# nv-tlabs/vid2player3d

Measured on AMD Instinct MI355X. Metric: env-steps/sec at num_envs=8192, SMPL humanoid imitation, higher is better.
Workload: dtype f32

## Files before the change

vid2player3d_amd/csrc/physics_ll.hip:

```cpp
#include <hip/hip_runtime.h>
#include <math.h>
#include <stdlib.h>
#include <string.h>

#if !defined(V2P_LL_STRICT_MATH)
#if !defined(V2P_LL_PRECISE_SINCOS)
#define PHYS_SINCOS(x, s, c) do { (s) = __sinf(x); (c) = __cosf(x); } while (0)
#endif
#if !defined(V2P_LL_PRECISE_SQRT)
#define PHYS_SQRT(x) __builtin_amdgcn_sqrtf(x)
#endif
#if !defined(V2P_LL_PRECISE_RCP)
#define PHYS_RCP(x) __builtin_amdgcn_rcpf(x)
#endif
#endif
#include "phys_common.hpp"
#include "hull_gjk.hpp"

#if defined(V2P_LL_REGS_BUILD)
#define V2P_LL_NS ll_regs
#define V2P_LL_LAUNCHER launch_env_physics_ll_regs
#else
#define V2P_LL_NS ll_lds
#define V2P_LL_LAUNCHER launch_env_physics_ll
#endif

namespace v2p {

#include "strict_ops.inc"

typedef volatile __attribute__((address_space(3))) float lds_vfloat;
constexpr int LPE = 32;

__device__ __forceinline__ bool any64(bool p) { return __builtin_amdgcn_ballot_w64(p) != 0ull; }
__device__ __forceinline__ uint8_t flag_ld(const uint8_t* p) { return __hip_atomic_load(p, __ATOMIC_RELAXED, __HIP_MEMORY_SCOPE_SYSTEM); }
__device__ __forceinline__ void flag_st(uint8_t* p, uint8_t v) { __hip_atomic_store(p, v, __ATOMIC_RELAXED, __HIP_MEMORY_SCOPE_SYSTEM); }
__device__ __forceinline__ float cload(const float* p) { return __hip_atomic_load(p, __ATOMIC_RELAXED, __HIP_MEMORY_SCOPE_SYSTEM); }
__device__ __forceinline__ void cstore(float* p, float v) { __hip_atomic_store(p, v, __ATOMIC_RELAXED, __HIP_MEMORY_SCOPE_SYSTEM); }
typedef float f4 __attribute__((ext_vector_type(4)));
__device__ __forceinline__ void cstore4(float* p, float x, float y, float z, float w) {
    const f4 v{x, y, z, w};
    asm volatile("global_store_dwordx4 %0, %1, off sc0 sc1\n\ts_nop 1" ::"v"(p), "v"(v) : "memory");
}
__device__ __forceinline__ void cload4x2(const float* p0, const float* p1, f4& a, f4& b) {
    asm volatile("global_load_dwordx4 %0, %2, off sc0 sc1\n\tglobal_load_dwordx4 %1, %3, off sc0 sc1\n\ts_waitcnt vmcnt(0)" : "=&v"(a), "=&v"(b) : "v"(p0), "v"(p1) : "memory");
}

__device__ __forceinline__ float pull(float v, int src_lane) {
    return __int_as_float(__builtin_amdgcn_ds_bpermute(src_lane << 2, __float_as_int(v)));
}
__device__ __forceinline__ V3 pull(V3 v, int s) { return V3{pull(v.x, s), pull(v.y, s), pull(v.z, s)}; }
__device__ __forceinline__ Q4 pull(Q4 q, int s) { return Q4{pull(q.x, s), pull(q.y, s), pull(q.z, s), pull(q.w, s)}; }
__device__ __forceinline__ Sym3 pull(const Sym3& a, int s) {
    return Sym3{pull(a.xx, s), pull(a.xy, s), pull(a.xz, s), pull(a.yy, s), pull(a.yz, s), pull(a.zz, s)};
}
__device__ __forceinline__ M3 pull(const M3& a, int s) {
    M3 r;
#pragma unroll
    for (int i = 0; i < 9; ++i) r.m[i] = pull(a.m[i], s);
    return r;
}
__device__ __forceinline__ float from_next(float v) { return __int_as_float(__builtin_amdgcn_update_dpp(0, __float_as_int(v), 0x130, 0xf, 0xf, true)); }
__device__ __forceinline__ V3 from_next(V3 v) { return V3{from_next(v.x), from_next(v.y), from_next(v.z)}; }
__device__ __forceinline__ Sym3 from_next(const Sym3& a) {
    return Sym3{from_next(a.xx), from_next(a.xy), from_next(a.xz), from_next(a.yy), from_next(a.yz), from_next(a.zz)};
}
__device__ __forceinline__ M3 from_next(const M3& a) {
    M3 r;
#pragma unroll
    for (int i = 0; i < 9; ++i) r.m[i] = from_next(a.m[i]);
    return r;
}
struct ParentPull {
    int plane;
    bool chain;
    __device__ __forceinline__ float operator()(float v, bool nonchain) const {
        return pull(v, plane);
    }
    __device__ __forceinline__ V3 operator()(V3 v, bool nonchain) const {
        return V3{pull(v.x, plane), pull(v.y, plane), pull(v.z, plane)};
    }
    __device__ __forceinline__ Q4 operator()(Q4 q, bool nonchain) const {
        return Q4{pull(q.x, plane), pull(q.y, plane), pull(q.z, plane), pull(q.w, plane)};
    }
    __device__ __forceinline__ Sym3 operator()(const Sym3& a, bool nonchain) const {
        return Sym3{pull(a.xx, plane), pull(a.xy, plane), pull(a.xz, plane), pull(a.yy, plane), pull(a.yz, plane), pull(a.zz, plane)};
    }
    __device__ __forceinline__ M3 operator()(const M3& a, bool nonchain) const {
        M3 r;
#pragma unroll
        for (int i = 0; i < 9; ++i) r.m[i] = pull(a.m[i], plane);
        return r;
    }
};
__device__ __forceinline__ Sym3 operator+(const Sym3& a, const Sym3& b) {
    return Sym3{a.xx + b.xx, a.xy + b.xy, a.xz + b.xz, a.yy + b.yy, a.yz + b.yz, a.zz + b.zz};
}
__device__ __forceinline__ Sym3 mask(bool c, const Sym3& a) {
    return Sym3{c ? a.xx : 0.f, c ? a.xy : 0.f, c ? a.xz : 0.f, c ? a.yy : 0.f, c ? a.yz : 0.f, c ? a.zz : 0.f};
}
__device__ __forceinline__ V3 mask(bool c, V3 a) { return V3{c ? a.x : 0.f, c ? a.y : 0.f, c ? a.z : 0.f}; }

__device__ __forceinline__ unsigned grp_xor1(unsigned v) { return (unsigned)__builtin_amdgcn_update_dpp(0, (int)v, 0xB1, 0xf, 0xf, false); }
__device__ __forceinline__ unsigned grp_xor2(unsigned v) { return (unsigned)__builtin_amdgcn_update_dpp(0, (int)v, 0x4E, 0xf, 0xf, false); }
__device__ __forceinline__ unsigned grp_mirror(unsigned v) { return (unsigned)__builtin_amdgcn_update_dpp(0, (int)v, 0x141, 0xf, 0xf, false); }
template <bool MAX, typename F>
__device__ __forceinline__ void grp_arg_step(float& v, int& k, F xch) {
    const float ov = __uint_as_float(xch(__float_as_uint(v)));
    const int ok = (int)xch((unsigned)k);
    const bool beats = MAX ? ov > v : ov < v;
    const bool take = ok >= 0 && (k < 0 || beats || (ov == v && ok < k));
    v = take ? ov : v;
    k = take ? ok : k;
}
__device__ __forceinline__ void grp_argmin(float& v, int& k) {
    grp_arg_step<false>(v, k, grp_xor1); grp_arg_step<false>(v, k, grp_xor2); grp_arg_step<false>(v, k, grp_mirror);
}
__device__ __forceinline__ void grp_argmax(float& v, int& k) {
    grp_arg_step<true>(v, k, grp_xor1); grp_arg_step<true>(v, k, grp_xor2); grp_arg_step<true>(v, k, grp_mirror);
}
__device__ __forceinline__ float grp_fmin(float v) {
    v = fminf(v, __uint_as_float(grp_xor1(__float_as_uint(v)))); v = fminf(v, __uint_as_float(grp_xor2(__float_as_uint(v)))); v = fminf(v, __uint_as_float(grp_mirror(__float_as_uint(v))));
    return v;
}
__device__ __forceinline__ float grp_fmax(float v) {
    v = fmaxf(v, __uint_as_float(grp_xor1(__float_as_uint(v)))); v = fmaxf(v, __uint_as_float(grp_xor2(__float_as_uint(v)))); v = fmaxf(v, __uint_as_float(grp_mirror(__float_as_uint(v))));
    return v;
}
__device__ __forceinline__ unsigned grp_umin(unsigned v) {
    unsigned o = grp_xor1(v); v = o < v ? o : v; o = grp_xor2(v); v = o < v ? o : v; o = grp_mirror(v); v = o < v ? o : v;
    return v;
}
template <bool MAX, bool FAST>
__device__ __forceinline__ void grp_arg(float& v, int& k) {
    if (!FAST) {
        if (MAX) grp_argmax(v, k); else grp_argmin(v, k);
        return;
    }
    const float m = k < 0 ? (MAX ? -3.0e38f : 3.0e38f) : v;
    const float g = MAX ? grp_fmax(m) : grp_fmin(m);
    const unsigned c = grp_umin((k >= 0 && m == g) ? (unsigned)k : 0x7fffffffu);
    k = c == 0x7fffffffu ? -1 : (int)c;
    v = g;
}

#define LLSUBV(k, tv) do { if (DIAG && a.prof) { long long t_ = clock64(); if (((a.prof_heavy ? blockIdx.x < 8u : (blockIdx.x & 63) == 0)) && lane == 0) atomicAdd((unsigned long long*)&a.prof[k], (unsigned long long)(t_ - tv)); tv = t_; } } while (0)
#define LLSUB(k) LLSUBV(k, tsub)
#ifdef V2P_LL_REGS_BUILD
#define LLSUBX(k, tv) do { } while (0)
#define LLSUBX_OR(k, kparent) LLSUB(kparent)
#define V2P_LL_DIAGX false
#else
#define LLSUBX(k, tv) LLSUBV(k, tv)
#define LLSUBX_OR(k, kparent) LLSUB(k)
#define V2P_LL_DIAGX DIAG
#endif
#define LLPH(k) do { if (DIAG && a.prof) { long long t_ = clock64(); if (((a.prof_heavy ? blockIdx.x < 8u : (blockIdx.x & 63) == 0)) && lane == 0) atomicAdd((unsigned long long*)&a.prof[k], (unsigned long long)(t_ - tprev)); tprev = t_; } } while (0)

inline namespace V2P_LL_NS {
#ifndef V2P_LL_WPS
#define V2P_LL_WPS 3
#endif
#ifndef V2P_LL_WPS_BALL
#define V2P_LL_WPS_BALL 3
#endif
#ifndef V2P_LL_WPS_LIMITS
#define V2P_LL_WPS_LIMITS 3
#endif
constexpr int LL_WPB = V2P_LL_WPB;
#ifndef V2P_LL_PARK2
#define V2P_LL_PARK2 1
#endif
constexpr bool PARK2 = V2P_LL_PARK2 != 0;
#ifndef V2P_LL_PARK3
#define V2P_LL_PARK3 1
#endif
constexpr bool PARK3 = V2P_LL_PARK3 != 0;
#ifndef V2P_LL_WAIT_SLEEP
#define V2P_LL_WAIT_SLEEP 16
#endif
constexpr int PARK_TAR = 0, PARK_W0 = 3, PARK_XD0 = 6, PARK_Q = 9, PARK_X = 13, PARK_CR = 16, PARK_CB = 28, PARK_CL = 32,
              PARK_SCR = PARK3 ? 44 : 16,
              PARK_SLOTS = PARK_SCR + 1;
constexpr int ROOTLAM_FLOATS = 2 * 24;
constexpr int BL_POS = 0, BL_QUAT = 3, BL_VEL = 7, BL_ANG = 10, BL_F = 13, BL_GA = 16, BL_GGAP = 17, BL_GBIAS = 18, BL_GLAM = 19, BL_GREST = 22, BL_RK = 24,
              RK_A = 0, RK_GAP = 1, RK_BIAS = 2, RK_RL = 3, RK_N = 6, RK_LAM = 9, RK_LINK = 12, RK_REST = 13, NBREC = 5, BL_V0 = BL_RK + 16 * NBREC, BL_SLOTS = BL_V0 + 8;
constexpr int LDS_FLOATS_PER_WAVE = PARK_SLOTS * 64 + 2 * BL_SLOTS + ROOTLAM_FLOATS;
__device__ __noinline__ f4 ball_hull_distance(ConstShape* S, int v0, int nv, V3 c) {
    V3 p;
    const float d = hull_closest([&](int k) { return V3{S->hull_verts[v0 + k][0], S->hull_verts[v0 + k][1], S->hull_verts[v0 + k][2]}; }, nv, c, p);
    return f4{p.x, p.y, p.z, d};
}
template <bool LDS>
struct ContactStore;
template <>
struct ContactStore<false> {
    V3 r_[4];
    float b_[4];
    V3 l_[4];
    __device__ __forceinline__ explicit ContactStore(float*) {}
    __device__ __forceinline__ V3 cr(int c) const { return r_[c]; }
    __device__ __forceinline__ void set_cr(int c, V3 v) { r_[c] = v; }
    __device__ __forceinline__ float bias(int c) const { return b_[c]; }
    __device__ __forceinline__ void set_bias(int c, float v) { b_[c] = v; }
    __device__ __forceinline__ V3 lam(int c) const { return l_[c]; }
    __device__ __forceinline__ void set_lam(int c, V3 v) { l_[c] = v; }
};
template <>
struct ContactStore<true> {
    float* p;
    __device__ __forceinline__ explicit ContactStore(float* park) : p(park) {}
    __device__ __forceinline__ V3 cr(int c) const { return V3{p[(PARK_CR + 3 * c) * 64], p[(PARK_CR + 3 * c + 1) * 64], p[(PARK_CR + 3 * c + 2) * 64]}; }
    __device__ __forceinline__ void set_cr(int c, V3 v) { p[(PARK_CR + 3 * c) * 64] = v.x; p[(PARK_CR + 3 * c + 1) * 64] = v.y; p[(PARK_CR + 3 * c + 2) * 64] = v.z; }
    __device__ __forceinline__ float bias(int c) const { return p[(PARK_CB + c) * 64]; }
    __device__ __forceinline__ void set_bias(int c, float v) { p[(PARK_CB + c) * 64] = v; }
    __device__ __forceinline__ V3 lam(int c) const { return V3{p[(PARK_CL + 3 * c) * 64], p[(PARK_CL + 3 * c + 1) * 64], p[(PARK_CL + 3 * c + 2) * 64]}; }
    __device__ __forceinline__ void set_lam(int c, V3 v) { p[(PARK_CL + 3 * c) * 64] = v.x; p[(PARK_CL + 3 * c + 1) * 64] = v.y; p[(PARK_CL + 3 * c + 2) * 64] = v.z; }
};

__device__ __forceinline__ void vfric_frame(const V3& w0, const V3& xd0, const V3& rr, V3& t1, V3& t2) {
    const float vx = xd0.x + w0.y * rr.z - w0.z * rr.y, vy = xd0.y + w0.z * rr.x - w0.x * rr.z;
    const float s2 = vx * vx + vy * vy;
    const bool on = s2 > 1e-12f;
    const float inv = on ? rsqrtf(s2) : 0.f;
    t1 = on ? V3{vx * inv, vy * inv, 0.f} : V3{1.f, 0.f, 0.f};
    t2 = V3{-t1.y, t1.x, 0.f};
}
template <bool CONTACT, bool MULTI, bool TGS, bool DIAG, bool BALL, bool JOBS, bool LIMITS, bool VFRIC = false>
__global__ __launch_bounds__(64 * LL_WPB, DIAG ? 2 : (BALL ? V2P_LL_WPS_BALL : (LIMITS ? V2P_LL_WPS_LIMITS : V2P_LL_WPS))) void physics_ll_kernel(PhysArgs a) {
    constexpr bool OPAQUE_H = BALL || LIMITS;
    const int64_t N = a.n;
    const int lane = threadIdx.x & 63;
    const int half = lane >> 5;
    const int lb = lane & (LPE - 1);
    const bool valid = lb < NB;
    const int b = valid ? lb : 0;
    const int base = lane & LPE;
    const int nblk = JOBS ? a.job_blocks : (int)gridDim.x;
    const int jid = (int)blockIdx.x;
    const bool mono = !JOBS || jid < a.job_mono;
    const int jcut = JOBS && nblk > a.job_mono ? nblk - a.job_mono : 1;
    const int jrel = JOBS ? jid - a.job_mono : 0;
    const int sjob = mono ? 0 : jrel / jcut;
    int jpair = jrel % jcut;
    if (JOBS && !mono && a.job_interleave) {
        const int nmix = a.pl_mix > a.job_mono ? (a.pl_mix < nblk ? a.pl_mix : nblk) - a.job_mono : 0;
        const int neq = jcut - nmix, both = 2 * (nmix < neq ? nmix : neq);
        if (jpair < both) jpair = (jpair & 1) ? nmix + (jpair >> 1) : (jpair >> 1);
        else jpair = nmix < neq ? jpair : jpair - neq;
    }
    const int bid = mono ? jid : a.job_mono + jpair;
    const int64_t slot = ((int64_t)bid * LL_WPB + (threadIdx.x >> 6)) * 2 + half;
    const bool live_env = slot < N;
    const int jlen = JOBS ? a.job_len : 1;
    const int jlead = JOBS ? a.job_lead : 1;
    auto jstart = [&](int j) -> int { return j <= 0 ? 0 : jlead + (j - 1) * jlen; };
    const bool first_job = mono || sjob == 0, last_job = mono || jstart(sjob + 1) >= a.p.nsub;
    bool handed = !mono && sjob > 0;
    int* const progress = JOBS ? a.job_progress + (bid * LL_WPB + (threadIdx.x >> 6)) : nullptr;
    if constexpr (JOBS) if (!mono) {
        int done = 0;
        if (lane == 0) done = __hip_atomic_load(progress, __ATOMIC_RELAXED, __HIP_MEMORY_SCOPE_SYSTEM) >= a.job_epoch * (a.p.nsub + 1) + a.p.nsub;
        if (__builtin_amdgcn_readfirstlane(done)) {
            if (lane == 0 && half == 0) __hip_atomic_fetch_add(a.job_progress + a.job_blocks * LL_WPB + 1, 1, __ATOMIC_RELAXED, __HIP_MEMORY_SCOPE_SYSTEM);
            return;
        }
    }
    auto wait_for_predecessor = [&]() {
    if constexpr (JOBS) if (handed) {
        const int want = a.job_epoch * (a.p.nsub + 1) + sjob;
        int ok = 1;
        if (lane == 0) {
            long spins = 0;
            while (__hip_atomic_load(progress, __ATOMIC_RELAXED, __HIP_MEMORY_SCOPE_SYSTEM) < want) {
                if (spins >= a.job_timeout_spins) {
                    ok = 0;
                    __hip_atomic_fetch_add(a.job_progress + a.job_blocks * LL_WPB, 1, __ATOMIC_RELAXED, __HIP_MEMORY_SCOPE_SYSTEM);
                    break;
                }
                __builtin_amdgcn_s_sleep(V2P_LL_WAIT_SLEEP);
                ++spins;
            }
        }
        handed = __builtin_amdgcn_readfirstlane(ok) != 0;
        __builtin_amdgcn_wave_barrier();
    }
    };
    wait_for_predecessor();
    int64_t e = live_env ? slot : N - 1;
    if (a.pl_start && handed) {
        e = __hip_atomic_load(&a.pl_slot_env[live_env ? slot : N - 1], __ATOMIC_RELAXED, __HIP_MEMORY_SCOPE_SYSTEM);
    } else if (a.pl_start) {
        const int nn = (int)N, mixn = a.pl_mix;
        const int64_t sl0 = ((int64_t)bid * LL_WPB + (threadIdx.x >> 6)) * 2;
        const int s0 = (int)(sl0 < N ? sl0 : N - 1), s1 = (int)(sl0 + 1 < N ? sl0 + 1 : N - 1);
        const int r0 = s0 < 2 * mixn ? ((s0 & 1) ? nn - 1 - (s0 >> 1) : (s0 >> 1)) : s0 - mixn;
// ... 603 lines not shown
#endif
                int* const scr = (int*)(park_all + (threadIdx.x >> 6) * LDS_FLOATS_PER_WAVE + PARK_SCR * 64);
                if (near) scr[myk] = lane;
                if (DIAG && a.prof && ((a.prof_heavy ? blockIdx.x < 8u : (blockIdx.x & 63) == 0)) && lane == 0) atomicAdd((unsigned long long*)&a.prof[13], (unsigned long long)rounds);
                for (int rd = 0; rd < rounds; ++rd) {
                    const int kk = 8 * rd + grp;
                    const bool gon = kk < ntot;
                    const int src = gon ? scr[kk] : lane;
                    const M3 RL = q2mat(pull(q, src));
                    const V3 xL = pull(x, src);
                    const float r6 = RL.m[6], r7 = RL.m[7], r8 = RL.m[8], xz = xL.z;
                    const int v0L = __builtin_amdgcn_ds_bpermute(src << 2, v0), nvL = __builtin_amdgcn_ds_bpermute(src << 2, nv);
                    ConstShape* const SL = MULTI ? (ConstShape*)(a.shapes + __builtin_amdgcn_ds_bpermute(src << 2, sid)) : S;
                    auto hullv = [&](int idx) -> float4 { return make_float4(SL->hull_verts[idx][0], SL->hull_verts[idx][1], SL->hull_verts[idx][2], 0.f); };
                    const float r0 = RL.m[0], r1 = RL.m[1], r2 = RL.m[2], xx = xL.x;
                    const float r3 = RL.m[3], r4 = RL.m[4], r5 = RL.m[5], xy = xL.y;
                    const unsigned gbit = 1u << gl;
                    float4 vv[8];
#pragma unroll
                    for (int k = 0; k < 8; ++k) {
                        const int i = 8 * k + gl;
                        vv[k] = hullv(v0L + ((gon && i < nvL) ? i : 0));
                    }
                    float px[8], py[8];
                    unsigned clo = 0u, chi = 0u;
                    int k0 = -1;
                    float zmin = 0.f;
#pragma unroll
                    for (int k = 0; k < 8; ++k) {
                        const int i = 8 * k + gl;
                        const bool in = gon && i < nvL;
                        const float z = xz + r6 * vv[k].x + r7 * vv[k].y + r8 * vv[k].z;
                        px[k] = xx + r0 * vv[k].x + r1 * vv[k].y + r2 * vv[k].z;
                        py[k] = xy + r3 * vv[k].x + r4 * vv[k].y + r5 * vv[k].z;
                        const bool c = in && (z < coff);
                        const unsigned bit = c ? gbit << (8 * (k & 3)) : 0u;
                        if (k < 4) clo |= bit; else chi |= bit;
                        const bool better = c && (k0 < 0 || z < zmin);
                        k0 = better ? i : k0;
                        zmin = better ? z : zmin;
                    }
                    clo |= grp_xor1(clo); chi |= grp_xor1(chi);
                    clo |= grp_xor2(clo); chi |= grp_xor2(chi);
                    clo |= grp_mirror(clo); chi |= grp_mirror(chi);
                    grp_arg<false, FASTARG>(zmin, k0);
                    const unsigned long long cm = ((unsigned long long)chi << 32) | clo;
                    const int cntg = __popc(clo) + __popc(chi);
                    unsigned long long t = cm;
                    int s0 = t ? __ffsll((long long)t) - 1 : -1; t &= t - 1;
                    int s1 = t ? __ffsll((long long)t) - 1 : -1; t &= t - 1;
                    int s2 = t ? __ffsll((long long)t) - 1 : -1; t &= t - 1;
                    int s3 = t ? __ffsll((long long)t) - 1 : -1;
                    int ns = cntg < 4 ? cntg : 4;
                    const bool big = gon && cntg > 4;
                    if (any64(big)) {
                        if (DIAG && a.prof && ((a.prof_heavy ? blockIdx.x < 8u : (blockIdx.x & 63) == 0)) && lane == 0) atomicAdd((unsigned long long*)&a.prof[15], 1ull);
                        const int k0s = k0 < 0 ? 0 : k0;
                        const float4 u0 = hullv(v0L + k0s);
                        const float p0x = xx + r0 * u0.x + r1 * u0.y + r2 * u0.z;
                        const float p0y = xy + r3 * u0.x + r4 * u0.y + r5 * u0.z;
                        const unsigned long long remB = big ? (cm & ~(1ull << k0s)) : 0ull;
                        const unsigned blo = (unsigned)remB, bhi = (unsigned)(remB >> 32);
                        int k1 = -1;
                        float best = -1.f;
#pragma unroll
                        for (int k = 0; k < 8; ++k) {
                            const bool on = ((k < 4 ? blo : bhi) & (gbit << (8 * (k & 3)))) != 0u;
                            const float dx = px[k] - p0x, dy = py[k] - p0y;
                            const float d2 = dx * dx + dy * dy;
                            const bool take = on && (d2 > best);
                            best = take ? d2 : best;
                            k1 = take ? 8 * k + gl : k1;
                        }
                        grp_arg<true, FASTARG>(best, k1);
                        const int k1s = k1 < 0 ? 0 : k1;
                        const float4 u1 = hullv(v0L + k1s);
                        const float ex = xx + r0 * u1.x + r1 * u1.y + r2 * u1.z - p0x;
                        const float ey = xy + r3 * u1.x + r4 * u1.y + r5 * u1.z - p0y;
                        const unsigned long long remC = remB & ~(1ull << k1s);
                        const unsigned elo = (unsigned)remC, ehi = (unsigned)(remC >> 32);
                        int k2 = -1, k3 = -1;
                        float amax = 0.f, amin = 0.f;
#pragma unroll
                        for (int k = 0; k < 8; ++k) {
                            const bool on = ((k < 4 ? elo : ehi) & (gbit << (8 * (k & 3)))) != 0u;
                            const float dx = px[k] - p0x, dy = py[k] - p0y;
                            const float area = ex * dy - ey * dx;
                            const bool up = on && area > amax;
                            const bool dn = on && area < amin;
                            amax = up ? area : amax; k2 = up ? 8 * k + gl : k2;
                            amin = dn ? area : amin; k3 = dn ? 8 * k + gl : k3;
                        }
                        grp_arg<true, FASTARG>(amax, k2);
                        grp_arg<false, FASTARG>(amin, k3);
                        if (big) {
                            s0 = k0; s1 = k1;
                            s2 = k2 >= 0 ? k2 : k3;
                            s3 = k2 >= 0 ? k3 : -1;
                            ns = 2 + (k2 >= 0 ? 1 : 0) + (k3 >= 0 ? 1 : 0);
                        }
                    }
                    const int gpack = (s0 & 0x7f) | ((s1 & 0x7f) << 7) | ((s2 & 0x7f) << 14) | ((s3 & 0x7f) << 21) | (ns << 28);
                    const int got = __builtin_amdgcn_ds_bpermute(((myk & 7) << 3) << 2, gpack);
                    pack = (near && (myk >> 3) == rd) ? got : pack;
                }
            }
            LLSUB(17);
            int sel4[4];
#pragma unroll
            for (int c = 0; c < 4; ++c) {
                const int sv = (pack >> (7 * c)) & 0x7f;
                sel4[c] = sv == 0x7f ? -1 : sv;
            }
            cnt = (pack >> 28) & 7;
            if (any64(cnt > 0)) {
                const M3 R = q2mat(q);
                const float ih = 1.f / h;
#pragma unroll
                for (int c = 0; c < 4; ++c) {
                    const float4 uu = hullv(v0 + (sel4[c] < 0 ? 0 : sel4[c]));
                    const V3 crc = mul(R, V3{uu.x, uu.y, uu.z});
                    CS.set_cr(c, crc);
                    float dz = x.z + crc.z - P.rest_offset;
                    CS.set_bias(c, TGS ? dz : (dz >= 0.f ? dz * ih : fmaxf(P.erp * dz * ih, -P.max_depen)));
                }
            }
            if (a.contact_ids && last && valid && live_env && !frozen) {
#pragma unroll
                for (int c = 0; c < 4; ++c) a.contact_ids[(env_here() * NB + b) * 4 + c] = c < cnt ? b * 64 + sel4[c] : -1;
            }
            if (a.contact_ids_sub && valid && live_env && !frozen) {
#pragma unroll
                for (int c = 0; c < 4; ++c) a.contact_ids_sub[((env_here() * nsub + sub) * NB + b) * 4 + c] = c < cnt ? b * 64 + sel4[c] : -1;
            }

            LLSUB(18);
            if (PARK2 && lb == 0) {
                float lv[21];
#pragma unroll
                for (int k = 0; k < 21; ++k) lv[k] = rootlam[k];
                Lam.A = Sym3{lv[0], lv[1], lv[2], lv[3], lv[4], lv[5]};
#pragma unroll
                for (int k = 0; k < 9; ++k) Lam.B.m[k] = lv[6 + k];
                Lam.C = Sym3{lv[15], lv[16], lv[17], lv[18], lv[19], lv[20]};
            }
            auto ball_rec_mine = [&](int j) -> bool { return j < 2 ? racket_lane : lb == (int)bl[BL_RK + 16 * j + RK_LINK]; };
            bool myhull = false;
            if (BALL) {
#pragma unroll
                for (int j = 2; j < NBREC; ++j) myhull = myhull || (bl[BL_RK + 16 * j + RK_A] != 0.f && lb == (int)bl[BL_RK + 16 * j + RK_LINK]);
            }
            const bool ballhit = BALL && valid && ((racket_lane && (bl[BL_RK + RK_A] != 0.f || bl[BL_RK + 16 + RK_A] != 0.f)) || myhull);
            const bool ballground = BALL && ball_lane && bl[BL_GA] != 0.f;
            const unsigned long long tb = __ballot(valid && (cnt > 0 || ballhit));
            const unsigned m0 = (unsigned)tb, m1 = (unsigned)(tb >> 32);
            if (LIMITS && any64(limact)) {
                const V3 wv = PARK2 ? park_get3(PARK_W0) : w;
                const V3 pwv = pp(wv, true);
                const V3 om = mulT(q2mat(q), wv - pwv);
                const float mrate = P.limit_margin * PHYS_RCP(h);
                const float lscale = TGS ? PHYS_RCP(h) : 1.f;
                bool anyrow = false;
#pragma unroll
                for (int i = 0; i < 3; ++i) {
                    const float omi = i == 0 ? om.x : (i == 1 ? om.y : om.z);
                    const bool on = lsgn[i] != 0.f && lbias[i] * lscale < mrate + fmaxf(0.f, -lsgn[i] * omi);
                    if (!on) lsgn[i] = 0.f;
                    anyrow = anyrow || on;
                }
                limact = anyrow;
            }
            const unsigned long long lmb = LIMITS ? __ballot(valid && limact) : 0ull;
            const unsigned lm0 = (unsigned)lmb, lm1 = (unsigned)(lmb >> 32);
            if (DIAG && a.wave_times) { const int tt = __popc(half ? m1 : m0); tsum += tt; tmaxs = tt > tmaxs ? tt : tmaxs; }
            if (last) {
                const unsigned mine = half ? m1 : m0;
                ksum = __popc(mine);
                kdep = 0;
                for (unsigned t = mine; t; t &= t - 1) { const int dd = M.depth[__ffs(t) - 1]; kdep = dd > kdep ? dd : kdep; }
            }
            if (DIAG && a.prof && ((a.prof_heavy ? blockIdx.x < 8u : (blockIdx.x & 63) == 0)) && lane == 0) { atomicAdd((unsigned long long*)&a.prof[9], (unsigned long long)(__popc(m0) + __popc(m1))); atomicAdd((unsigned long long*)&a.prof[10], 1ull); }
            const bool sweep_on = ((m0 | m1 | lm0 | lm1) || (BALL && any64(ballground))) && P.n_iter > 0;
            if (PARK2 && !sweep_on) unpark_vel(w, xd);
            if (sweep_on) {
                int dn0 = 0, dn1 = 0;
                for (unsigned t = m0 | lm0; t; t &= t - 1) { const int dd = M.depth[__ffs(t) - 1]; dn0 = dd > dn0 ? dd : dn0; }
                for (unsigned t = m1 | lm1; t; t &= t - 1) { const int dd = M.depth[__ffs(t) - 1]; dn1 = dd > dn1 ? dd : dn1; }
                const int dneed = dn0 > dn1 ? dn0 : dn1, dmin = dn0 < dn1 ? dn0 : dn1;
                const bool insweep = dep <= (half ? dn1 : dn0);
                LLPH(4);
                for (int d = 1; d <= dneed; ++d) {
                    Blocks Lp;
                    const bool nc = (nonchain >> d) & 1;
                    Lp.A = pp(Lam.A, nc);
                    Lp.B = pp(Lam.B, nc);
                    Lp.C = pp(Lam.C, nc);
                    if (dep == d) {
                        V3 la0{Lp.A.xx, Lp.A.xy, Lp.A.xz}, la1{Lp.A.xy, Lp.A.yy, Lp.A.yz}, la2{Lp.A.xz, Lp.A.yz, Lp.A.zz};
                        M3 Gb;
                        {
                            V3 g0 = cross(la0, r) + row(Lp.B, 0), g1 = cross(la1, r) + row(Lp.B, 1), g2 = cross(la2, r) + row(Lp.B, 2);
                            Gb.m[0] = g0.x; Gb.m[1] = g0.y; Gb.m[2] = g0.z; Gb.m[3] = g1.x; Gb.m[4] = g1.y; Gb.m[5] = g1.z; Gb.m[6] = g2.x; Gb.m[7] = g2.y; Gb.m[8] = g2.z;
                        }
                        Sym3 Gc;
                        {
                            V3 q0 = cross(col(Gb, 0), r), q1 = cross(col(Gb, 1), r), q2 = cross(col(Gb, 2), r);
                            V3 n0 = cross(r, col(Lp.B, 0)), n1 = cross(r, col(Lp.B, 1)), n2 = cross(r, col(Lp.B, 2));
                            Gc.xx = Lp.C.xx + q0.x - n0.x;
                            Gc.xy = Lp.C.xy + q0.y - n1.x;
                            Gc.xz = Lp.C.xz + q0.z - n2.x;
                            Gc.yy = Lp.C.yy + q1.y - n1.y;
                            Gc.yz = Lp.C.yz + q1.z - n2.y;
                            Gc.zz = Lp.C.zz + q2.z - n2.z;
                        }
                        M3 DiM;
                        DiM.m[0] = Di.xx; DiM.m[1] = Di.xy; DiM.m[2] = Di.xz; DiM.m[3] = Di.xy; DiM.m[4] = Di.yy; DiM.m[5] = Di.yz; DiM.m[6] = Di.xz; DiM.m[7] = Di.yz; DiM.m[8] = Di.zz;
                        M3 H1, H2;
#pragma unroll
                        for (int i = 0; i < 3; ++i) {
                            V3 gai = i == 0 ? la0 : (i == 1 ? la1 : la2);
                            V3 gbi = row(Gb, i);
                            V3 gbti = col(Gb, i);
                            V3 gci = i == 0 ? V3{Gc.xx, Gc.xy, Gc.xz} : (i == 1 ? V3{Gc.xy, Gc.yy, Gc.yz} : V3{Gc.xz, Gc.yz, Gc.zz});
#pragma unroll
                            for (int j = 0; j < 3; ++j) {
                                V3 dj = col(DiM, j);
                                V3 ej = row(E, j);
                                H1.m[3 * i + j] = aug * dot(gai, dj) - dot(gbi, ej);
                                H2.m[3 * i + j] = aug * dot(gbti, dj) - dot(gci, ej);
                            }
                        }
                        M3 t;
#pragma unroll
                        for (int i = 0; i < 3; ++i)
#pragma unroll
                            for (int j = 0; j < 3; ++j) t.m[3 * i + j] = aug * dot(row(DiM, i), col(H1, j)) - dot(row(E, i), col(H2, j));
                        Lam.A = Sym3{Di.xx + t.m[0], Di.xy + 0.5f * (t.m[1] + t.m[3]), Di.xz + 0.5f * (t.m[2] + t.m[6]), Di.yy + t.m[4],
                                     Di.yz + 0.5f * (t.m[5] + t.m[7]), Di.zz + t.m[8]};
#pragma unroll
                        for (int i = 0; i < 3; ++i)
#pragma unroll
                            for (int j = 0; j < 3; ++j) {
                                V3 gcj = j == 0 ? V3{Gc.xx, Gc.xy, Gc.xz} : (j == 1 ? V3{Gc.xy, Gc.yy, Gc.yz} : V3{Gc.xz, Gc.yz, Gc.zz});
                                Lam.B.m[3 * i + j] = aug * dot(row(DiM, i), col(Gb, j)) - dot(row(E, i), gcj);
                            }
                        Lam.C = Gc;
                        if (LIMITS && limact) {
                            const Sym3 K{Lam.A.xx - 2.f * H1.m[0] + Lp.A.xx, Lam.A.xy - H1.m[1] - H1.m[3] + Lp.A.xy, Lam.A.xz - H1.m[2] - H1.m[6] + Lp.A.xz,
                                         Lam.A.yy - 2.f * H1.m[4] + Lp.A.yy, Lam.A.yz - H1.m[5] - H1.m[7] + Lp.A.yz, Lam.A.zz - 2.f * H1.m[8] + Lp.A.zz};
                            const M3 R = q2mat(Q4{park[PARK_Q * 64], park[(PARK_Q + 1) * 64], park[(PARK_Q + 2) * 64], park[(PARK_Q + 3) * 64]});
                            const V3 c0 = col(R, 0), c1 = col(R, 1), c2 = col(R, 2);
                            const V3 k0 = mul(K, c0), k1 = mul(K, c1), k2 = mul(K, c2);
                            Kd = Sym3{dot(c0, k0), dot(c0, k1), dot(c0, k2), dot(c1, k1), dot(c1, k2), dot(c2, k2)};
                        }
                    }
                }

                auto ball_dirs = [&](V3 n, V3& t1, V3& t2) {
                    t1 = cross(n, V3{0.f, 0.f, 1.f});
                    if (dot(t1, t1) < 1e-6f) t1 = cross(n, V3{1.f, 0.f, 0.f});
                    t1 = rsqrtf(dot(t1, t1)) * t1;
                    t2 = cross(n, t1);
                };
                if (PARK2) unpark_vel(w, xd);
                if (BALL && ballhit) {
                    const V3 bv{bl[BL_VEL], bl[BL_VEL + 1], bl[BL_VEL + 2]}, bw{bl[BL_ANG], bl[BL_ANG + 1], bl[BL_ANG + 2]};
                    const float ih = PHYS_RCP(h);
#pragma unroll
                    for (int j = 0; j < NBREC; ++j) {
                        lds_vfloat* rk = bl + BL_RK + 16 * j;
                        if (rk[RK_A] != 0.f && ball_rec_mine(j)) {
                            const V3 n{rk[RK_N], rk[RK_N + 1], rk[RK_N + 2]}, rl{rk[RK_RL], rk[RK_RL + 1], rk[RK_RL + 2]};
                            const float gap = rk[RK_GAP];
                            const float vn0 = dot(bv + cross(bw, -BP.radius * n) - xd - cross(w, rl), n);
                            float bias = gap >= 0.f ? gap * ih : fmaxf(P.erp * gap * ih, -P.max_depen);
                            const float rest = (vn0 < -BP.bounce_thr && gap * ih + vn0 < 0.f) ? (j < 2 ? BP.rest_racket : BP.rest_body) * vn0 : 3.0e38f;
                            bias = fminf(bias, rest);
                            rk[RK_BIAS] = bias;
                            if (TGS) rk[RK_REST] = rest;
                        }
                    }
                }
                LLPH(5);
                if (!PARK2) {
                    park_put3(PARK_W0, w);
                    park_put3(PARK_XD0, xd);
                }
                [[maybe_unused]] unsigned chain0 = 0u, chain1 = 0u;
                {
                    int prev = -1;
                    for (unsigned t = m0; t; t &= t - 1) {
                        const int nn = __ffs(t) - 1;
                        if ((int)((a.par_pack[nn / 12] >> (5 * (nn % 12))) & 31ull) == prev) chain0 |= 1u << nn;
                        prev = nn;
                    }
                    prev = -1;
                    for (unsigned t = m1; t; t &= t - 1) {
                        const int nn = __ffs(t) - 1;
                        if ((int)((a.par_pack[nn / 12] >> (5 * (nn % 12))) & 31ull) == prev) chain1 |= 1u << nn;
                        prev = nn;
                    }
                    chain0 &= ~lm0;
                    chain1 &= ~lm1;
                }
                const float hs = h / (float)P.n_iter;
                float tgs_irem = 1.f / h;
                const float tgs_pen = P.erp / hs;
                auto rowbias = [&](float v) -> float { return TGS ? (v >= 0.f ? v * tgs_irem : fmaxf(tgs_pen * v, -P.max_depen)) : v; };
                V3 un_tot{0.f, 0.f, 0.f}, un_new{0.f, 0.f, 0.f}, uf_new{0.f, 0.f, 0.f}, Dw{0.f, 0.f, 0.f}, Dv{0.f, 0.f, 0.f};
                int cur0 = 0, cur1 = 0;
                bool live0 = false, live1 = false;
                const unsigned v0 = LIMITS ? m0 | lm0 : m0, v1 = LIMITS ? m1 | lm1 : m1;
                V3 jt_new{0.f, 0.f, 0.f};
#ifdef V2P_LL_REGS_BUILD
                constexpr bool VTAB = !LIMITS && !TGS && !BALL && !DIAG;
#else
                constexpr bool VTAB = !LIMITS && !TGS && !BALL;
#endif
                constexpr bool LIVEM = VTAB;
#ifdef V2P_LL_REGS_BUILD
                constexpr bool ROWX = VTAB;
#else
                constexpr bool ROWX = true;
#endif
                constexpr bool ROWCNT = ROWX && VTAB;
                int minfo = 0;
                [[maybe_unused]] int vis = 0, mystop = -1, nvis0 = 0, nvis1 = 0;
                [[maybe_unused]] int livem = 0;
                [[maybe_unused]] unsigned anc = 0u;
                {
                    int p0 = v0 ? 31 - __clz(v0) : 0, p1 = v1 ? 31 - __clz(v1) : 0;
                    if constexpr (VTAB) {
                        nvis0 = __popc(v0);
                        nvis1 = __popc(v1);
                    }
                    int k = 0;
                    for (unsigned s0 = v0, s1 = v1; s0 | s1; s0 &= s0 - 1, s1 &= s1 - 1, ++k) {
                        const int b0 = s0 ? __ffs(s0) - 1 : p0, b1 = s1 ? __ffs(s1) - 1 : p1;
                        const int selp = half ? p1 : p0, selb = half ? b1 : b0;
                        const bool ap = valid && ((desc >> selp) & 1), ab = valid && ((desc >> selb) & 1);
                        const unsigned long long bp = __ballot(ap), bb = __ballot(ab), bc = __ballot(ap && ab);
                        const int du = __popc(half ? (unsigned)(bp >> 32) : (unsigned)bp) - 1, dn = __popc(half ? (unsigned)(bb >> 32) : (unsigned)bb) - 1,
                                  dl = __popc(half ? (unsigned)(bc >> 32) : (unsigned)bc) - 1;
                        const int sd = (half ? M.side_depths[p1] : M.side_depths[p0]) & ~((2 << dl) - 1);
                        if constexpr (VTAB) {
                            const bool has = (half ? s1 : s0) != 0u;
                            int np = 0;
                            if constexpr (ROWCNT) { const int c0 = __builtin_amdgcn_readlane(cnt, b0), c1 = __builtin_amdgcn_readlane(cnt, 32 + b1); np = (half ? c1 : c0) << 25; }
                            if (has && lb == k) vis = dl | (du << 4) | (dn << 8) | ((sd & 0xfff) << 12) | ((half ? nvis1 : nvis0) > 1 ? 1 << 24 : 0) | np;
                            if (has && valid && lb == selb) mystop = k;
                            if (has && ab) anc |= 2u << k;
                            if (k == 0 && ap) anc |= 1u;
                        } else {
                            if (valid && lb == selb && ((half ? s1 : s0) != 0u)) minfo = dl | (du << 4) | (dn << 8) | (sd << 12) | ((LIMITS && !firstchild) ? 1 << 28 : 0);
                        }
                        p0 = b0;
                        p1 = b1;
                    }
                }
                if constexpr (VTAB) {
                    cur0 = v0 ? 31 - __clz(v0) : 0;
                    cur1 = v1 ? 31 - __clz(v1) : 0;
                }
                constexpr bool UPMASK = !LIMITS && !TGS;
                [[maybe_unused]] int vk = 0;
                auto walk_to = [&](int nx0, int nx1, int info0, int info1, bool mv0, bool mv1) {
                    long long tsub = DIAG && a.prof ? clock64() : 0;
                    const int pk0 = __builtin_amdgcn_readfirstlane(mv0 ? info0 : 0x00f), pk1 = __builtin_amdgcn_readfirstlane(mv1 ? info1 : 0x00f);
                    const int dl0 = pk0 & 15, dn0 = (pk0 >> 8) & 15;
                    const int dl1 = pk1 & 15, dn1 = (pk1 >> 8) & 15;
                    const int selc = half ? cur1 : cur0, seln = half ? nx1 : nx0, mydl = half ? dl1 : dl0;
                    const bool onc = VTAB ? ((anc >> vk) & 1u) != 0u : valid && ((desc >> selc) & 1), onn = VTAB ? ((anc >> vk) & 2u) != 0u : valid && ((desc >> seln) & 1);
                    int uk0 = pk0, uk1 = pk1;
                    if constexpr (LIMITS) {
                        const bool pend = onc && dep > mydl && (un_new.x != 0.f || un_new.y != 0.f || un_new.z != 0.f || uf_new.x != 0.f || uf_new.y != 0.f || uf_new.z != 0.f ||
                                                                jt_new.x != 0.f || jt_new.y != 0.f || jt_new.z != 0.f);
                        const unsigned long long pb = __ballot(pend);
                        uk0 = __builtin_amdgcn_readfirstlane((unsigned)pb ? pk0 : 0x00f);
                        uk1 = __builtin_amdgcn_readfirstlane((unsigned)(pb >> 32) ? pk1 : 0x00f);
                    }
                    const int du0 = (uk0 >> 4) & 15, du1 = (uk1 >> 4) & 15, ul0 = uk0 & 15, ul1 = uk1 & 15, myul = half ? ul1 : ul0;
                    const int updep = (onc && dep > myul) ? dep : -1, dndep = (onn && dep > mydl) ? dep : -1;
                    const int turndep = (onc && dep == myul) ? dep : -2;
                    const int ulmin = ul0 < ul1 ? ul0 : ul1, dlmin = dl0 < dl1 ? dl0 : dl1;
                    const unsigned sideb = ((unsigned)(uk0 >> 12) | (unsigned)(uk1 >> 12)) & 0xfffu;
                    if constexpr (UPMASK) {
                        const int dmax = du0 > du1 ? du0 : du1;
                        if (dmax > ulmin) {
                            const int rcdep = onc ? dep + 1 : -1;
                            const int ucl1 = has1 ? cl1 : base + 31, ucl2 = has2 ? cl2 : base + 31;
                            V3 cn, cf, rn{0.f, 0.f, 0.f}, rf{0.f, 0.f, 0.f};
                            asm("" : "=v"(cn.x), "=v"(cn.y), "=v"(cn.z), "=v"(cf.x), "=v"(cf.y), "=v"(cf.z));
                            for (int dctr = dmax; dctr > ulmin; --dctr) {
                                int d = dctr;
                                asm volatile("" : "+s"(d));
                                if (updep == d) {
                                    const float axx = aug * Di.xx, axy = aug * Di.xy, axz = aug * Di.xz, ayy = aug * Di.yy, ayz = aug * Di.yz, azz = aug * Di.zz;
                                    const V3 na{__builtin_fmaf(un_new.x, axx, __builtin_fmaf(un_new.y, axy, un_new.z * axz)),
                                                __builtin_fmaf(un_new.x, axy, __builtin_fmaf(un_new.y, ayy, un_new.z * ayz)),
                                                __builtin_fmaf(un_new.x, axz, __builtin_fmaf(un_new.y, ayz, un_new.z * azz))};
                                    const V3 fa{uf_new.x - __builtin_fmaf(un_new.x, E.m[0], __builtin_fmaf(E.m[3], un_new.y, E.m[6] * un_new.z)),
                                                uf_new.y - __builtin_fmaf(un_new.x, E.m[1], __builtin_fmaf(E.m[4], un_new.y, E.m[7] * un_new.z)),
                                                uf_new.z - __builtin_fmaf(un_new.x, E.m[2], __builtin_fmaf(E.m[5], un_new.y, E.m[8] * un_new.z))};
                                    cn = V3{__builtin_fmaf(fa.z, r.y, __builtin_fmaf(-r.z, fa.y, na.x)), __builtin_fmaf(-r.x, fa.z, __builtin_fmaf(fa.x, r.z, na.y)),
                                            __builtin_fmaf(fa.y, r.x, __builtin_fmaf(-r.y, fa.x, na.z))};
                                    cf = fa;
                                    un_new = V3{0.f, 0.f, 0.f};
                                    uf_new = V3{0.f, 0.f, 0.f};
                                }
                                if (updep == d || rcdep == d) {
                                    rn = from_next(cn);
                                    rf = from_next(cf);
                                    if ((sideb >> d) & 1u) {
                                        rn = rn + pull(cn, ucl1) + pull(cn, ucl2);
                                        rf = rf + pull(cf, ucl1) + pull(cf, ucl2);
                                    }
                                    un_new = un_new + rn;
                                    uf_new = uf_new + rf;
                                    un_tot = un_tot + rn;
                                }
                            }
                            if (turndep >= 0) {
                                Dw = Dw + mul(Lam.A, rn) + mul(Lam.B, rf);
                                Dv = Dv + V3{dot(col(Lam.B, 0), rn), dot(col(Lam.B, 1), rn), dot(col(Lam.B, 2), rn)} + mul(Lam.C, rf);
                            }
                        }
                    } else {
                        const unsigned longb = sideb | (ul0 < 15 ? 2u << ul0 : 0u) | (ul1 < 15 ? 2u << ul1 : 0u);
                        for (int dctr = du0 > du1 ? du0 : du1; dctr > ulmin; --dctr) {
                            int d = dctr;
                            asm volatile("" : "+s"(d));
                            V3 cn{0.f, 0.f, 0.f}, cf{0.f, 0.f, 0.f};
                            if (updep == d) {
                                const V3 na = aug * mul(Di, un_new);
                                const V3 fa = uf_new - V3{dot(col(E, 0), un_new), dot(col(E, 1), un_new), dot(col(E, 2), un_new)};
                                cn = na + cross(r, fa);
                                cf = fa;
                                un_new = V3{0.f, 0.f, 0.f};
                                uf_new = V3{0.f, 0.f, 0.f};
                                if (LIMITS) {
                                    cn = cn - jt_new;
                                    jt_new = V3{0.f, 0.f, 0.f};
                                }
                            }
                            if (!((longb >> d) & 1u)) {
                                un_new = un_new + from_next(cn);
                                uf_new = uf_new + from_next(cf);
                                un_tot = un_tot + from_next(cn);
                            } else {
                                V3 rn = from_next(mask(firstchild, cn)), rf = from_next(mask(firstchild, cf));
                                if ((sideb >> d) & 1u) {
                                    rn = rn + mask(has1, pull(cn, cl1)) + mask(has2, pull(cn, cl2));
                                    rf = rf + mask(has1, pull(cf, cl1)) + mask(has2, pull(cf, cl2));
                                }
                                un_new = un_new + rn;
                                uf_new = uf_new + rf;
                                un_tot = un_tot + rn;
                                if (turndep == d - 1) {
                                    Dw = Dw + mul(Lam.A, rn) + mul(Lam.B, rf);
                                    Dv = Dv + V3{dot(col(Lam.B, 0), rn), dot(col(Lam.B, 1), rn), dot(col(Lam.B, 2), rn)} + mul(Lam.C, rf);
                                }
                            }
                        }
                    }
                    LLSUB(12);
                    const int dtop = dn0 > dn1 ? dn0 : dn1;
                    for (int d = dlmin + 1; d <= dtop; ++d) {
                        const bool nc = (nonchain >> d) & 1;
                        const V3 pdw = pp(Dw, nc), pdv = pp(Dv, nc);
                        if (dndep == d) {
                            const V3 tv = pdv + cross(pdw, r);
                            Dw = mul(Di, aug * pdw + un_tot) - mul(E, tv);
                            Dv = tv;
                        }
                    }
                    LLSUB(14);
                };
                auto walk_close = [&](int dlast, bool all) {
                    [[maybe_unused]] long long tclose = V2P_LL_DIAGX && a.prof ? clock64() : 0;
                    const int i0 = ((int)__builtin_amdgcn_readlane(dep, cur0) << 4) | (M.side_depths[cur0] << 12);
                    const int i1 = ((int)__builtin_amdgcn_readlane(dep, 32 + cur1) << 4) | (M.side_depths[cur1] << 12);
                    const int slive = LIVEM ? livem : __builtin_amdgcn_readfirstlane((live0 ? 1 : 0) | (live1 ? 2 : 0));
                    vk = 0;
                    [[maybe_unused]] const long long tmove = V2P_LL_DIAGX && a.prof ? clock64() : 0;
                    walk_to(0, 0, i0, i1, (slive & 1) != 0, (slive & 2) != 0);
                    if (V2P_LL_DIAGX && a.prof) {
                        const long long tdone = clock64();
                        if (((a.prof_heavy ? blockIdx.x < 8u : (blockIdx.x & 63) == 0)) && lane == 0) atomicAdd((unsigned long long*)&a.prof[12], (unsigned long long)(tmove - tdone));
                    }
                    LLSUBX(20, tclose);
                    long long tsub = DIAG && a.prof ? clock64() : 0;
                    V3 ddw{0.f, 0.f, 0.f}, ddv{0.f, 0.f, 0.f};
                    if (lb == 0) {
                        ddw = Dw;
                        ddv = Dv;
                        w = w + ddw;
                        xd = xd + ddv;
                    }
                    for (int d = 1; d <= dlast; ++d) {
                        const bool nc = (nonchain >> d) & 1;
                        const V3 pdw = pp(ddw, nc), pdv = pp(ddv, nc);
                        if (dep == d && (all || insweep)) {
                            const V3 av = pdv + cross(pdw, r);
                            ddw = mul(Di, aug * pdw + un_tot) - mul(E, av);
                            ddv = av;
                            w = w + ddw;
                            xd = xd + ddv;
                        }
// ... 696 lines not shown
```

Before: 23.06 million.

## Replace serial per-link depth scans and visit-table setup with DPP reductions and precomputed masks

In the common configuration without limits, TGS or ball, the maximum depth of touched links is computed with a DPP max-reduction over each 32-lane half, replacing serial loops that read depth from the table for each set bit. The visit-table setup also changes. Each visited lane now writes its own row entry into scratch LDS using precomputed ancestor masks and popcounts, and the ancestor bits come from readlane plus inverse_ballot. This replaces the per-visit loop that issued three ballots per iteration. It removes serialized scalar work in front of the sweep, at the cost of new scratch LDS traffic and a dependence on the anc_mask metadata being consistent with the old ballot-derived values.

After: 23.48 million, median of 6. +1.9%, better.

```diff
diff --git a/vid2player3d_amd/csrc/physics_ll.hip b/vid2player3d_amd/csrc/physics_ll.hip
--- a/vid2player3d_amd/csrc/physics_ll.hip
+++ b/vid2player3d_amd/csrc/physics_ll.hip
@@ -142,6 +142,15 @@
     const unsigned c = grp_umin((k >= 0 && m == g) ? (unsigned)k : 0x7fffffffu);
     k = c == 0x7fffffffu ? -1 : (int)c;
     v = g;
+}
+
+__device__ __forceinline__ int half_max_last(int v) {
+    int o = __builtin_amdgcn_update_dpp(0, v, 0x111, 0xf, 0xf, true); v = o > v ? o : v;
+    o = __builtin_amdgcn_update_dpp(0, v, 0x112, 0xf, 0xf, true); v = o > v ? o : v;
+    o = __builtin_amdgcn_update_dpp(0, v, 0x114, 0xf, 0xf, true); v = o > v ? o : v;
+    o = __builtin_amdgcn_update_dpp(0, v, 0x118, 0xf, 0xf, true); v = o > v ? o : v;
+    o = __builtin_amdgcn_update_dpp(0, v, 0x142, 0xa, 0xf, false); v = o > v ? o : v;
+    return v;
 }
 
 #define LLSUBV(k, tv) do { if (DIAG && a.prof) { long long t_ = clock64(); if (((a.prof_heavy ? blockIdx.x < 8u : (blockIdx.x & 63) == 0)) && lane == 0) atomicAdd((unsigned long long*)&a.prof[k], (unsigned long long)(t_ - tv)); tv = t_; } } while (0)
@@ -1051,7 +1060,8 @@
             }
             const bool ballhit = BALL && valid && ((racket_lane && (bl[BL_RK + RK_A] != 0.f || bl[BL_RK + 16 + RK_A] != 0.f)) || myhull);
             const bool ballground = BALL && ball_lane && bl[BL_GA] != 0.f;
-            const unsigned long long tb = __ballot(valid && (cnt > 0 || ballhit));
+            const bool touched = valid && (cnt > 0 || ballhit);
+            const unsigned long long tb = __ballot(touched);
             const unsigned m0 = (unsigned)tb, m1 = (unsigned)(tb >> 32);
             if (LIMITS && any64(limact)) {
                 const V3 wv = PARK2 ? park_get3(PARK_W0) : w;
@@ -1072,19 +1082,39 @@
             const unsigned long long lmb = LIMITS ? __ballot(valid && limact) : 0ull;
             const unsigned lm0 = (unsigned)lmb, lm1 = (unsigned)(lmb >> 32);
             if (DIAG && a.wave_times) { const int tt = __popc(half ? m1 : m0); tsum += tt; tmaxs = tt > tmaxs ? tt : tmaxs; }
+#ifdef V2P_LL_REGS_BUILD
+            constexpr bool SETUPX = !LIMITS && !TGS && !BALL && !DIAG;
+#else
+            constexpr bool SETUPX = !LIMITS && !TGS && !BALL;
+#endif
+            [[maybe_unused]] int tdep0 = 0, tdep1 = 0;
+            if constexpr (SETUPX) {
+                const int tdred = half_max_last(touched ? dep : 0);
+                tdep0 = __builtin_amdgcn_readlane(tdred, 31);
+                tdep1 = __builtin_amdgcn_readlane(tdred, 63);
+            }
             if (last) {
                 const unsigned mine = half ? m1 : m0;
                 ksum = __popc(mine);
-                kdep = 0;
-                for (unsigned t = mine; t; t &= t - 1) { const int dd = M.depth[__ffs(t) - 1]; kdep = dd > kdep ? dd : kdep; }
+                if constexpr (SETUPX) {
+                    kdep = half ? tdep1 : tdep0;
+                } else {
+                    kdep = 0;
+                    for (unsigned t = mine; t; t &= t - 1) { const int dd = M.depth[__ffs(t) - 1]; kdep = dd > kdep ? dd : kdep; }
+                }
             }
             if (DIAG && a.prof && ((a.prof_heavy ? blockIdx.x < 8u : (blockIdx.x & 63) == 0)) && lane == 0) { atomicAdd((unsigned long long*)&a.prof[9], (unsigned long long)(__popc(m0) + __popc(m1))); atomicAdd((unsigned long long*)&a.prof[10], 1ull); }
             const bool sweep_on = ((m0 | m1 | lm0 | lm1) || (BALL && any64(ballground))) && P.n_iter > 0;
             if (PARK2 && !sweep_on) unpark_vel(w, xd);
             if (sweep_on) {
                 int dn0 = 0, dn1 = 0;
-                for (unsigned t = m0 | lm0; t; t &= t - 1) { const int dd = M.depth[__ffs(t) - 1]; dn0 = dd > dn0 ? dd : dn0; }
-                for (unsigned t = m1 | lm1; t; t &= t - 1) { const int dd = M.depth[__ffs(t) - 1]; dn1 = dd > dn1 ? dd : dn1; }
+                if constexpr (SETUPX) {
+                    dn0 = tdep0;
+                    dn1 = tdep1;
+                } else {
+                    for (unsigned t = m0 | lm0; t; t &= t - 1) { const int dd = M.depth[__ffs(t) - 1]; dn0 = dd > dn0 ? dd : dn0; }
+                    for (unsigned t = m1 | lm1; t; t &= t - 1) { const int dd = M.depth[__ffs(t) - 1]; dn1 = dd > dn1 ? dd : dn1; }
+                }
                 const int dneed = dn0 > dn1 ? dn0 : dn1, dmin = dn0 < dn1 ? dn0 : dn1;
                 const bool insweep = dep <= (half ? dn1 : dn0);
                 LLPH(4);
@@ -1185,8 +1215,8 @@
                     park_put3(PARK_W0, w);
                     park_put3(PARK_XD0, xd);
                 }
-                [[maybe_unused]] unsigned chain0 = 0u, chain1 = 0u;
-                {
+                if constexpr (!SETUPX) {
+                    [[maybe_unused]] unsigned chain0 = 0u, chain1 = 0u;
                     int prev = -1;
                     for (unsigned t = m0; t; t &= t - 1) {
                         const int nn = __ffs(t) - 1;
@@ -1216,6 +1246,7 @@
 #else
                 constexpr bool VTAB = !LIMITS && !TGS && !BALL;
 #endif
+                static_assert(VTAB == SETUPX, "the set-up in front of the sweep and the table go together");
                 constexpr bool LIVEM = VTAB;
 #ifdef V2P_LL_REGS_BUILD
                 constexpr bool ROWX = VTAB;
@@ -1227,14 +1258,37 @@
                 [[maybe_unused]] int vis = 0, mystop = -1, nvis0 = 0, nvis1 = 0;
                 [[maybe_unused]] int livem = 0;
                 [[maybe_unused]] unsigned anc = 0u;
-                {
+                if constexpr (VTAB) {
+                    const unsigned mine = half ? v1 : v0;
+                    nvis0 = __popc(v0);
+                    nvis1 = __popc(v1);
+                    const int nmine = half ? nvis1 : nvis0;
+                    const unsigned below = mine & ((1u << lb) - 1u);
+                    const int kme = __popc(below);
+                    const int plast0 = v0 ? 31 - __clz(v0) : 0, plast1 = v1 ? 31 - __clz(v1) : 0;
+                    const unsigned ancme = valid ? (unsigned)M.anc_mask[bo] : 0u;
+                    int* const vrow = (int*)(park + PARK_SCR * 64);
+                    if (valid && ((mine >> lb) & 1u)) {
+                        const int pv = below ? 31 - __clz(below) : (half ? plast1 : plast0);
+                        const unsigned ancp = (unsigned)M.anc_mask[pv];
+                        const int sdp = M.side_depths[pv];
+                        const int du = __popc(ancp) - 1, dl = __popc(ancp & ancme) - 1;
+                        const int sd = sdp & ~((2 << dl) - 1);
+                        vrow[kme - lb] = dl | (du << 4) | (dep << 8) | ((sd & 0xfff) << 12) | (nmine > 1 ? 1 << 24 : 0) | (ROWCNT ? cnt << 25 : 0);
+                        mystop = kme;
+                    }
+                    vis = lb < nmine ? vrow[0] : 0;
+                    auto lanes_of = [&](unsigned lo, unsigned hi) -> bool { return __builtin_amdgcn_inverse_ballot_w64(((unsigned long long)hi << 32) | lo); };
+                    anc = lanes_of(__builtin_amdgcn_readlane(ancme, plast0), __builtin_amdgcn_readlane(ancme, 32 + plast1)) ? 1u : 0u;
+                    int k = 1;
+                    for (unsigned s0 = v0, s1 = v1; s0 | s1; s0 &= s0 - 1, s1 &= s1 - 1, ++k) {
+                        const unsigned a0 = __builtin_amdgcn_readlane(ancme, __ffs(s0 | 0x80000000u) - 1);
+                        const unsigned a1 = __builtin_amdgcn_readlane(ancme, 32 + __ffs(s1 | 0x80000000u) - 1);
+                        anc |= lanes_of(a0, a1) ? 1u << k : 0u;
+                    }
+                } else {
                     int p0 = v0 ? 31 - __clz(v0) : 0, p1 = v1 ? 31 - __clz(v1) : 0;
-                    if constexpr (VTAB) {
-                        nvis0 = __popc(v0);
-                        nvis1 = __popc(v1);
-                    }
-                    int k = 0;
-                    for (unsigned s0 = v0, s1 = v1; s0 | s1; s0 &= s0 - 1, s1 &= s1 - 1, ++k) {
+                    for (unsigned s0 = v0, s1 = v1; s0 | s1; s0 &= s0 - 1, s1 &= s1 - 1) {
                         const int b0 = s0 ? __ffs(s0) - 1 : p0, b1 = s1 ? __ffs(s1) - 1 : p1;
                         const int selp = half ? p1 : p0, selb = half ? b1 : b0;
                         const bool ap = valid && ((desc >> selp) & 1), ab = valid && ((desc >> selb) & 1);
@@ -1242,17 +1296,7 @@
                         const int du = __popc(half ? (unsigned)(bp >> 32) : (unsigned)bp) - 1, dn = __popc(half ? (unsigned)(bb >> 32) : (unsigned)bb) - 1,
                                   dl = __popc(half ? (unsigned)(bc >> 32) : (unsigned)bc) - 1;
                         const int sd = (half ? M.side_depths[p1] : M.side_depths[p0]) & ~((2 << dl) - 1);
-                        if constexpr (VTAB) {
-                            const bool has = (half ? s1 : s0) != 0u;
-                            int np = 0;
-                            if constexpr (ROWCNT) { const int c0 = __builtin_amdgcn_readlane(cnt, b0), c1 = __builtin_amdgcn_readlane(cnt, 32 + b1); np = (half ? c1 : c0) << 25; }
-                            if (has && lb == k) vis = dl | (du << 4) | (dn << 8) | ((sd & 0xfff) << 12) | ((half ? nvis1 : nvis0) > 1 ? 1 << 24 : 0) | np;
-                            if (has && valid && lb == selb) mystop = k;
-                            if (has && ab) anc |= 2u << k;
-                            if (k == 0 && ap) anc |= 1u;
-                        } else {
-                            if (valid && lb == selb && ((half ? s1 : s0) != 0u)) minfo = dl | (du << 4) | (dn << 8) | (sd << 12) | ((LIMITS && !firstchild) ? 1 << 28 : 0);
-                        }
+                        if (valid && lb == selb && ((half ? s1 : s0) != 0u)) minfo = dl | (du << 4) | (dn << 8) | (sd << 12) | ((LIMITS && !firstchild) ? 1 << 28 : 0);
                         p0 = b0;
                         p1 = b1;
                     }
```
